# GreatV/oar-ocr

Measured on AMD Instinct MI355X. Metric: images/sec end-to-end PP-OCRv6 det+rec, higher is better.
Workload: dtype f32; 1 GPU; PP-OCRv6-tiny-class det+rec (synthetic-weight graphs: det 447089 params, rec 1135700 params, V=6906), batch=32 synthetic 960x960 pages per GPU, 40 text lines/page; timed region = u8 pages in pageable HOST memory -> oar_ocr_predict -> oar_ocr_decode -> sorted boxes + texts + scores on the host; image_batch_size=32, region_batch_size=256, parallelism=image-parallel x1

## Files before the change

### oar_ocr_amd/build.py

```python
from __future__ import annotations

import os
import subprocess
import sys
from concurrent.futures import ThreadPoolExecutor
from pathlib import Path

HERE = Path(__file__).resolve().parent
CSRC = HERE / "csrc"
LIBDIR = HERE / "lib"
LIB = LIBDIR / "libOarMi355x.so"
SOURCES = ["common.cc", "onnx_parse.cc", "engine.cc", "db_host.cc", "poly_host.cc", "pipeline.cc", "c_api.cc", "ctc_host.cc", "image_decode.cc", "image_misc_decode.cc", "jpeg_decode.cc", "layout.cc", "kernels.hip", "igemm.hip", "igemm_ws_1x1.hip", "igemm_ws_gen.hip", "igemm_ws_x6.hip", "igemm_os_x6.hip", "igemm_ws3.hip", "igemm_rs3_x6.hip", "prepost.hip", "contours.hip", "jpeg.hip", "layout.hip", "dsblock.hip", "dsblock_k3s1.hip", "dsblock_k3s2.hip", "dsblock_k5s1.hip", "dsblock_k5s2.hip", "dsblock_wa_a.hip", "dsblock_wa_b.hip", "dsblock_rs_k3s11.hip", "dsblock_rs_k3s21.hip", "dsblock_rs_k3s12.hip", "dsblock_rs_k3s22.hip", "dsblock_rs_dbg.hip", "dsblock_cs.hip", "dsblock_pc.hip", "dsblock_rs2.hip", "ctc_head_x6.hip", "chain.hip", "attention_x6.hip", "igemm_lk_x6.hip", "index_ops.hip", "sla_decode.hip"]
HIPCC = os.environ.get("HIPCC", "/opt/rocm/bin/hipcc")
FLAGS = ["--offload-arch=gfx950", "-O3", "-std=c++17", "-fPIC", "-ffp-contract=off", "-fno-fast-math",
         "-Wno-unused-result", "-Wno-pass-failed"]
if os.environ.get("OAR_DSB_ABLATIONS"):
    FLAGS.append("-DOAR_DSB_ABLATIONS")


def _stale(out: Path, deps) -> bool:
    if not out.exists():
        return True
    t = out.stat().st_mtime
    return any(Path(d).stat().st_mtime > t for d in deps)


def build_lib(force: bool = False, verbose: bool = False) -> Path:
    LIBDIR.mkdir(exist_ok=True)
    objdir = LIBDIR / "obj"
    objdir.mkdir(exist_ok=True)
    headers = list(CSRC.glob("*.h")) + list(CSRC.glob("*.inc")) + [HERE.parent / "include" / "oar_mi355x.h"]
    jobs = []
    for s in SOURCES:
        src = CSRC / s
        obj = objdir / (s.replace(".", "_") + ".o")
        if force or _stale(obj, [src] + headers):
            jobs.append((src, obj))

    def cc(job):
        src, obj = job
        cmd = [HIPCC] + FLAGS + ["-c", str(src), "-o", str(obj)]
        if verbose:
            print(" ".join(cmd), flush=True)
        r = subprocess.run(cmd, capture_output=True, text=True)
        if r.returncode != 0:
# ... 28 lines not shown
```

### oar_ocr_amd/csrc/engine.cc

```cpp
#include "engine.h"

#include "dsblock.h"

#include <algorithm>
#include <cmath>
#include <cstring>
#include <set>
#include <sstream>

namespace oar {

using k::Act;

static int64_t numel(const std::vector<int64_t>& d) {
    int64_t n = 1;
    for (auto v : d) n *= v;
    return n;
}

Engine::Engine(const uint8_t* onnx, size_t len, int device_id, hipStream_t caller_stream) : device_(device_id) {
    int ndev = 0;
    if (hipGetDeviceCount(&ndev) != hipSuccess || ndev <= 0)
        fail(OAR_DEVICE, "no HIP device visible: libOarMi355x has no CPU fallback");
    OAR_CHECK(device_id >= 0 && device_id < ndev, OAR_DEVICE, "device_id out of range");
// ... 878 lines not shown
    std::vector<int64_t> s(d.size(), 1);
    for (int i = (int)d.size() - 2; i >= 0; --i) s[i] = s[i + 1] * d[i + 1];
    return s;
}

struct Planner {
    Engine& E;
    Plan& P;
    std::map<std::string, TInfo> vals;
    std::map<std::string, int> last_use;
    std::map<std::string, size_t> root_bytes;
    std::map<std::string, size_t> root_off;
    Arena arena;
    int cur = 0;
    std::vector<std::pair<size_t, size_t>> temps;

    Planner(Engine& e, Plan& p) : E(e), P(p) { opset = e.opset_; }

    struct PendingResize {
        Loc xin;
        std::vector<int64_t> dims;
        int N, H, W, C, Ho, Wo, imode, ictm, inm;
        float sh, sw;
        int fh = 0, fw = 0;
    };
    std::map<std::string, PendingResize> pending_resize;
    std::map<std::string, int> sole_consumer;
    void run_resize(const PendingResize& r, Loc yl, int64_t y_off, int y_ld) {
        const PendingResize q = r;
        step([=](const RunCtx& c) { k::resize(c.s, c.at(q.xin), c.mut(yl) + y_off, q.N, q.H, q.W, q.C, q.Ho, q.Wo, q.sh, q.sw, q.imode, q.ictm, q.inm, y_ld); }, 0,
             4.0 * ((double)q.N * q.H * q.W * q.C + (double)q.N * q.Ho * q.Wo * q.C));
    }
    std::map<std::string, const GNode*> pending_convt;
    struct PendingConcat { std::vector<Loc> src; std::vector<int> c; std::vector<int64_t> dims; };
    std::map<std::string, PendingConcat> pending_concat;
    std::map<std::string, int> concat_consumer;
    void emit_concat_gather(const PendingConcat& pc, Loc yl) {
        k::ConcatGatherP gp{};
        gp.n_src = (int)pc.src.size(); gp.N = (int)pc.dims[0]; gp.Ho = (int)pc.dims[2]; gp.Wo = (int)pc.dims[3]; gp.C = (int)pc.dims[1];
        int off = 0;
        for (size_t i = 0; i < pc.src.size(); ++i) { gp.c[i] = pc.c[i]; gp.off[i] = off; gp.fh[i] = 1; gp.fw[i] = 1; off += pc.c[i]; }
        const std::vector<Loc> src = pc.src;
        step([=](const RunCtx& c) {
            k::ConcatGatherP q = gp;
            for (int i = 0; i < q.n_src; ++i) q.x[i] = c.at(src[(size_t)i]);
            k::concat_gather(c.s, q, c.mut(yl));
        }, 0, 8.0 * (double)numel(pc.dims));
    }
    void materialise_concat(const std::string& name) {
        auto it = pending_concat.find(name);
        if (it == pending_concat.end()) return;
        const PendingConcat pc = it->second;
        pending_concat.erase(it);
        vals.erase(name);
        TInfo& y = new_out(name, pc.dims, Layout::CLAST);
        emit_concat_gather(pc, y.loc);
    }
    const PendingResize* peek_pending(const std::string& name) const {
        auto it = pending_resize.find(name);
        return it == pending_resize.end() ? nullptr : &it->second;
    }
    void materialise_pending(const std::string& name) {
        auto ct = pending_convt.find(name);
        if (ct != pending_convt.end()) {
            const GNode* node = ct->second;
            pending_convt.erase(ct);
            vals.erase(name);
            op_convt(*node, false);
            return;
        }
        auto it = pending_resize.find(name);
        if (it == pending_resize.end()) return;
        const PendingResize r = it->second;
        pending_resize.erase(it);
        TInfo& y = new_out(name, r.dims, Layout::CLAST);
        run_resize(r, y.loc, 0, r.C);
    }

    TInfo& get(const std::string& name) {
        if (!pending_resize.empty() || !pending_convt.empty()) materialise_pending(name);
// ... 613 lines not shown
            int64_t th = std::max<int64_t>((oh - 1) * sh + (kh - 1) * dh + 1 - H, 0), tw = std::max<int64_t>((ow - 1) * sw + (kw - 1) * dw + 1 - W, 0);
            if (ap == "SAME_UPPER") { pt = th / 2; pb = th - pt; pl = tw / 2; pr = tw - pl; }
            else { pb = th / 2; pt = th - pb; pr = tw / 2; pl = tw - pr; }
        }
    }

    void op_conv(const GNode& n) {
        if (n.in.size() > 3 && !n.in[3].empty()) {
            TInfo xg = get(n.in[0]), gt = get(n.in[3]);
            const TInfo& wg = get(n.in[1]);
            bool ok = xg.dims.size() == 4 && !xg.host_int && !gt.host_int && wg.ht && wg.ht->dims.size() == 4 && gt.loc.kind != Loc::NONE && n.residual.empty();
            if (ok) {
                const int64_t N = xg.dims[0], C = xg.dims[1], HW = xg.dims[2] * xg.dims[3];
                ok = numel(gt.dims) == N * C && gt.dims.size() >= 2 && gt.dims[0] == N && gt.dims[1] == C && wg.ht->dims[1] == C && C % 8 == 0 &&
                     k::conv_igemm_se_ok(N * HW, (int)C, (int)wg.ht->dims[0], (int)HW);
            }
            if (!ok) {
                GNode mul;
                mul.op = "Mul"; mul.in = {n.in[0], n.in[3]}; mul.out = {n.out[0] + "::se"};
                op_binary(mul, 2);
                GNode c2 = n;
                c2.in.resize(3);
                c2.in[0] = mul.out[0];
                op_conv(c2);
                return;
            }
        }
        PendingConcat msrc;
        {
            auto pit = pending_concat.find(n.in[0]);
            if (pit != pending_concat.end()) {
                auto wi = E.inits_.find(n.in.size() > 1 ? n.in[1] : std::string());
                const std::vector<int64_t>& pd = pit->second.dims;
                const bool still_ok = wi != E.inits_.end() && wi->second.dims.size() == 4 && wi->second.dims[2] == 1 && wi->second.dims[3] == 1 && n.residual.empty() &&
                                      !(n.in.size() > 3 && !n.in[3].empty()) && n.out.size() == 1 &&
                                      k::conv_msrc_ok((long)(pd[0] * pd[2] * pd[3]), (int)pd[1], (int)wi->second.dims[0]);
                if (getenv("OAR_DEBUG_CONCAT")) fprintf(stderr, "  conv %s reads pending concat: still_ok=%d (w4=%d res=%d gate=%d nout=%zu)\n", n.out[0].c_str(), (int)still_ok, (int)(wi != E.inits_.end() && wi->second.dims.size() == 4), (int)!n.residual.empty(), (int)(n.in.size() > 3 && !n.in[3].empty()), n.out.size());
                if (still_ok) { msrc = pit->second; TInfo keep = vals[n.in[0]]; pending_concat.erase(pit); vals[n.in[0]] = keep; }
            }
        }
        TInfo x = get(n.in[0]);
        OAR_CHECK(x.dims.size() == 4, OAR_UNSUPPORTED_OP, "Conv: only 2-D convolutions are supported");
        const TInfo& wt = get(n.in[1]);
        OAR_CHECK(wt.ht, OAR_UNSUPPORTED_OP, "Conv: weights must be an initializer");
        const HostTensor& W = *wt.ht;
        OAR_CHECK(W.dims.size() == 4 && W.dims[0] > 0 && W.dims[1] > 0 && W.dims[2] > 0 && W.dims[3] > 0, OAR_MODEL_LOAD, "Conv: weight must be rank 4 with positive dims at " + n.out[0]);
        int64_t N = x.dims[0], Cin = x.dims[1], H = x.dims[2], Wd = x.dims[3];
        int64_t Cout = W.dims[0], kh = W.dims[2], kw = W.dims[3], g = n.ai("group", 1);
        OAR_CHECK(g >= 1 && W.dims[1] * g == Cin && Cout % g == 0, OAR_SHAPE_MISMATCH, "Conv: weight/input channel mismatch at " + n.out[0]);
        if (has_input(n, 2)) { const TInfo& bt = get(n.in[2]); OAR_CHECK(bt.ht && (int64_t)bt.ht->f.size() == Cout, OAR_MODEL_LOAD, "Conv: bias must be an f32 initializer of Cout elements at " + n.out[0]); }
        auto st = n.ais("strides"), dl = n.ais("dilations");
        int64_t sh = st.size() == 2 ? st[0] : 1, sw = st.size() == 2 ? st[1] : 1;
        int64_t dh = dl.size() == 2 ? dl[0] : 1, dw = dl.size() == 2 ? dl[1] : 1;
        int64_t pt, pl, pb, pr;
        get_pads(n, H, Wd, kh, kw, sh, sw, dh, dw, pt, pl, pb, pr);
        int64_t Ho = (H + pt + pb - dh * (kh - 1) - 1) / sh + 1, Wo = (Wd + pl + pr - dw * (kw - 1) - 1) / sw + 1;
        if (x.u8_stem) {
            OAR_CHECK(g == 1 && Cin == 3 && kh * kw * 3 <= 128 && n.residual.empty(), OAR_INTERNAL, "run_stem on a graph whose first node is not an RGB stem");
            const float* sb = has_input(n, 2) ? get(n.in[2]).loc.cptr : nullptr;
            TInfo& ys = new_out(n.out[0], {N, Cout, Ho, Wo}, Layout::CLAST);
            k::ConvP sp{};
            sp.N = (int)N; sp.H = (int)H; sp.W = (int)Wd; sp.Cin = 3; sp.Ho = (int)Ho; sp.Wo = (int)Wo; sp.Cout = (int)Cout;
            sp.kh = (int)kh; sp.kw = (int)kw; sp.sh = (int)sh; sp.sw = (int)sw; sp.pt = (int)pt; sp.pl = (int)pl; sp.dh = (int)dh; sp.dw = (int)dw;
            sp.groups = 1; sp.act = n.act; sp.bias = sb; sp.y_ld = (int)Cout; sp.convt2x2 = 0;
            sp.w = conv_weight_direct(n, W);
            const Loc ysl = ys.loc;
            step([=](const RunCtx& c) {
// ... 98 lines not shown
            gate = get(n.in[3]).loc;
        }
        const bool has_gate = gate.kind != Loc::NONE;
        double flops = 2.0 * N * Ho * Wo * Cout * (Cin / g) * kh * kw;
        double bytes = 4.0 * (N * H * Wd * Cin + N * Ho * Wo * Cout * (has_res ? 2 : 1) + numel(W.dims));
        if (n.out.size() > 1) {
            const int tiles = kind == 1 ? k::conv_dw_gap_tiles(p) : 0;
            if (tiles > 0 && Cout <= 1024 && n.ai("gap_raw", 0) != 0) {
                TInfo& gy = new_out(n.out[1], {N, (int64_t)tiles * Cout, 1, 1}, Layout::CLAST);
                gy.gap_tiles = tiles; gy.gap_hw = (int)(Ho * Wo);
                const Loc part = gy.loc;
                step([=](const RunCtx& c) {
                    k::ConvP q = p;
                    q.x = c.at(xin); q.y = c.mut(yl); q.residual = has_res ? c.at(res) : nullptr; q.gap_part = c.mut(part);
                    k::conv_dw(c.s, q);
                }, flops, bytes + 4.0 * N * tiles * Cout);
                return;
            }
            if (tiles > 0 && Cout <= 1024) {
                TInfo& gy = new_out(n.out[1], {N, Cout, 1, 1}, Layout::CLAST);
                const Loc gl = gy.loc, part = alloc_temp((size_t)N * tiles * Cout * sizeof(float));
                const int hw = (int)(Ho * Wo);
                step([=](const RunCtx& c) {
                    k::ConvP q = p;
                    q.x = c.at(xin); q.y = c.mut(yl); q.residual = has_res ? c.at(res) : nullptr; q.gap_part = c.mut(part);
                    k::conv_dw(c.s, q);
                }, flops, bytes + 4.0 * N * tiles * Cout);
                step([=](const RunCtx& c) { k::global_avgpool_finish(c.s, c.at(part), c.mut(gl), (int)N, tiles, (int)Cout, hw); }, 0, 4.0 * N * tiles * Cout);
                return;
            }
        }
        const bool from_concat = !msrc.src.empty();
        OAR_CHECK(!from_concat || (kind == 0 && p.w_fmt == k::IGEMM_W_X6), OAR_INTERNAL, "Conv: deferred concat in front of a layer that is not on the bf16x6 kernels");
        auto run = [=](const RunCtx& c) {
            k::ConvP q = p;
            q.y = c.mut(yl); q.residual = has_res ? c.at(res) : nullptr; q.se = has_gate ? c.at(gate) : nullptr;
            if (from_concat) {
                q.x = nullptr; q.n_msrc = (int)msrc.src.size();
                for (int i = 0; i < q.n_msrc; ++i) { q.msrc[i] = c.at(msrc.src[(size_t)i]); q.msrc_c[i] = msrc.c[(size_t)i]; }
            } else {
                q.x = c.at(xin);
            }
            if (kind == 3) {
                const int ng = p.groups, cgi = p.Cin / ng, ogi = p.Cout / ng;
                for (int gi = 0; gi < ng; ++gi) {
                    k::ConvP r = q;
                    r.groups = 1; r.Cin = cgi; r.Cout = ogi; r.x_ld = p.Cin;
                    r.x = q.x + (size_t)gi * cgi; r.y = q.y + (size_t)gi * ogi; r.w = wgrp[(size_t)gi];
                    r.bias = q.bias ? q.bias + (size_t)gi * ogi : nullptr;
                    r.residual = q.residual ? q.residual + (size_t)gi * ogi : nullptr;
                    k::conv_igemm(c.s, r);
                }
                return;
            }
            if (kind == 4) {
                int c0 = 0;
                for (size_t i = 0; i < slices3.size(); ++i) {
                    k::ConvP r = q;
                    r.Cin = slices3[i]; r.x_ld = p.Cin; r.x = q.x + c0; r.w = wgrp[i]; r.accum = i > 0 ? 1 : 0;
                    if (i > 0) r.bias = nullptr;
                    if (i + 1 < slices3.size()) r.act = k::Act{};
                    k::conv_igemm(c.s, r);
                    c0 += slices3[i];
                }
                return;
            }
// ... 912 lines not shown
        }
        std::string mode = n.as("mode", "nearest"), ctm = n.as("coordinate_transformation_mode", "half_pixel"), nm = n.as("nearest_mode", "round_prefer_floor");
        int imode = mode == "nearest" ? 0 : 1;
        OAR_CHECK(mode == "nearest" || mode == "linear", OAR_UNSUPPORTED_OP, "Resize: mode " + mode);
        int ictm = ctm == "asymmetric" ? 0 : ctm == "half_pixel" ? 1 : ctm == "align_corners" ? 2 : ctm == "pytorch_half_pixel" ? 3 : -1;
        OAR_CHECK(ictm >= 0, OAR_UNSUPPORTED_OP, "Resize: coordinate_transformation_mode " + ctm);
        int inm = nm == "floor" ? 0 : nm == "round_prefer_floor" ? 1 : nm == "round_prefer_ceil" ? 2 : 3;
        static const bool defer_on = [] { const char* e = getenv("OAR_DEFER_RESIZE"); return !e || atoi(e) != 0; }();
        if (defer_on && imode == 0 && x.layout == Layout::CLAST && sole_consumer.count(n.out[0])) {
            PendingResize r;
            r.xin = x.loc; r.dims = {x.dims[0], x.dims[1], Ho, Wo};
            r.N = (int)x.dims[0]; r.H = (int)H; r.W = (int)W; r.C = (int)x.dims[1]; r.Ho = (int)Ho; r.Wo = (int)Wo;
            r.imode = imode; r.ictm = ictm; r.inm = inm; r.sh = sh; r.sw = sw;
            auto factor = [&](int in, int out, float scale) {
                if (in <= 0 || out % in != 0) return 0;
                const int f = out / in;
                for (int o = 0; o < out; ++o) if (k::resize_nearest_index(o, scale, in, out, ictm, inm) != o / f) return 0;
                return f;
            };
            r.fh = factor(r.H, r.Ho, sh); r.fw = factor(r.W, r.Wo, sw);
            if (!r.fh || !r.fw) r.fh = r.fw = 0;
            pending_resize[n.out[0]] = r;
            TInfo t;
            t.dims = r.dims; t.layout = Layout::CLAST; t.root = "";
            vals[n.out[0]] = t;
            return;
        }
        Loc xin = to_clast_loc(x);
        TInfo& y = new_out(n.out[0], {x.dims[0], x.dims[1], Ho, Wo}, Layout::CLAST);
        Loc yl = y.loc;
        int N = (int)x.dims[0], C = (int)x.dims[1];
        step([=](const RunCtx& c) { k::resize(c.s, c.at(xin), c.mut(yl), N, (int)H, (int)W, C, (int)Ho, (int)Wo, sh, sw, imode, ictm, inm, C); }, 0,
             4.0 * (numel(x.dims) + numel(y.dims)));
    }

    void op_concat(const GNode& n) {
        bool absorb = false;
        if (!pending_resize.empty()) {
            int64_t axis0 = n.ai("axis", 0);
            bool ok = true, any = false;
            int64_t total_c = 0;
            for (auto& s : n.in) {
                const PendingResize* pr = peek_pending(s);
                any = any || pr;
                auto it = vals.find(s);
                if (it == vals.end() || it->second.dims.size() != 4 || it->second.layout != Layout::CLAST || it->second.host_int) { ok = false; break; }
                if ((it->second.dims[1] & 3) != 0) ok = false;
                total_c += it->second.dims[1];
            }
            absorb = any && ok && (axis0 == 1 || axis0 == -3) && (total_c & 3) == 0;
            if (!absorb) for (auto& s : n.in) materialise_pending(s);
        }
        std::vector<TInfo> xs;
        for (auto& s : n.in) { auto it = vals.find(s); xs.push_back(absorb && peek_pending(s) ? it->second : get(s)); }
        bool all_host = true, any_host = false, any_f = false;
        for (auto& t : xs) { all_host = all_host && host_evaluable(t) && t.dims.size() <= 1; any_host = any_host || t.host_int; any_f = any_f || float_like(t); }
        if (all_host && any_host) {
            std::vector<double> v;
            for (auto& t : xs) { std::vector<double> e = host_values(t); v.insert(v.end(), e.begin(), e.end()); }
            set_host(n.out[0], {(int64_t)v.size()}, v, any_f);
            return;
        }
        int r = (int)xs[0].dims.size();
        int64_t axis = n.ai("axis", 0);
        if (axis < 0) axis += r;
        bool clast = false;
// ... 8 lines not shown
            for (int i = 0; i < pax; ++i) outer *= pod[i];
            for (int i = pax + 1; i < r; ++i) inner *= pod[i];
            std::vector<Loc> ins;
            for (size_t i = 0; i < xs.size(); ++i) ins.push_back(absorb && peek_pending(n.in[i]) ? Loc() : to_clast_loc(xs[i]));
            int64_t coff = 0, total = pod[pax] * inner;
            bool plain = !absorb && r == 4 && inner == 1 && xs.size() >= 3 && (od[1] & 3) == 0;
            for (auto& t : xs) plain = plain && t.dims.size() == 4 && (t.dims[1] & 3) == 0;
            static const bool defer_on = [] { const char* e = getenv("OAR_CONCAT_DEFER"); return !(e && e[0] == '0'); }();
            if (getenv("OAR_DEBUG_CONCAT")) fprintf(stderr, "concat %s: plain=%d absorb=%d r=%d inner=%ld n=%zu consumer=%d\n", n.out[0].c_str(), (int)plain, (int)absorb, r, (long)inner, xs.size(), concat_consumer.count(n.out[0]) ? concat_consumer[n.out[0]] : -1);
            if (plain && defer_on && xs.size() <= 8 && concat_consumer.count(n.out[0])) {
                const GNode& cn = E.nodes_[concat_consumer[n.out[0]]];
                auto wi = E.inits_.find(cn.in.size() > 1 ? cn.in[1] : std::string());
                auto attr_ok = [&](const char* a, int64_t want) { auto v = cn.ais(a); for (auto e : v) if (e != want) return false; return true; };
                bool ok = wi != E.inits_.end() && wi->second.dims.size() == 4 && wi->second.dims[2] == 1 && wi->second.dims[3] == 1 && wi->second.dims[1] == od[1] && cn.ai("group", 1) == 1 &&
                          attr_ok("strides", 1) && attr_ok("pads", 0) && attr_ok("dilations", 1) && cn.residual.empty() && !(cn.in.size() > 3 && !cn.in[3].empty()) &&
                          cn.as("auto_pad", "NOTSET") == "NOTSET";
                for (auto& t : xs) ok = ok && t.layout == Layout::CLAST && (t.dims[1] & 7) == 0 && t.dims[0] == od[0] && t.dims[2] == od[2] && t.dims[3] == od[3] && !t.host_int;
                if (getenv("OAR_DEBUG_CONCAT")) {
                    fprintf(stderr, "  ok before msrc check = %d (K=%ld N=%ld) res=%d gate=%d autopad=%s\n", (int)ok, (long)od[1], wi != E.inits_.end() ? (long)wi->second.dims[0] : -1L, (int)!cn.residual.empty(), (int)(cn.in.size() > 3 && !cn.in[3].empty()), cn.as("auto_pad", "NOTSET").c_str());
                    for (auto& t : xs) fprintf(stderr, "    src layout=%d C=%ld host=%d\n", (int)(t.layout == Layout::CLAST), (long)t.dims[1], (int)t.host_int);
                }
                ok = ok && k::conv_msrc_ok((long)(od[0] * od[2] * od[3]), (int)od[1], (int)wi->second.dims[0]) && (wi->second.dims[0] & 3) == 0;
                if (ok) {
                    PendingConcat pc;
                    for (size_t i = 0; i < xs.size(); ++i) { pc.src.push_back(ins[i]); pc.c.push_back((int)xs[i].dims[1]); }
                    pc.dims = od;
                    TInfo t;
                    t.dims = od; t.layout = Layout::CLAST;
                    vals[n.out[0]] = t;
                    pending_concat[n.out[0]] = std::move(pc);
                    return;
                }
            }
            TInfo& y = new_out(n.out[0], od, Layout::CLAST);
            Loc yl = y.loc;
            if ((absorb || plain) && r == 4 && inner == 1 && xs.size() <= 8) {
                static const bool gather_on = [] { const char* e = getenv("OAR_CONCAT_GATHER"); return !(e && e[0] == '0'); }();
                bool ok = gather_on;
                for (size_t i = 0; ok && i < xs.size(); ++i) {
                    const PendingResize* pr = peek_pending(n.in[i]);
                    if (pr) ok = pr->fh > 0 && pr->fw > 0 && pr->imode == 0 && pr->Ho == od[2] && pr->Wo == od[3] && pr->H * pr->fh == pr->Ho && pr->W * pr->fw == pr->Wo && pr->N == od[0];
                    else ok = xs[i].dims[0] == od[0] && xs[i].dims[2] == od[2] && xs[i].dims[3] == od[3];
                }
                if (ok) {
                    k::ConcatGatherP gp{};
                    std::vector<Loc> src(xs.size());
                    gp.n_src = (int)xs.size(); gp.N = (int)od[0]; gp.Ho = (int)od[2]; gp.Wo = (int)od[3]; gp.C = (int)od[1];
                    double bytes = 4.0 * (double)numel(od);
                    for (size_t i = 0; i < xs.size(); ++i) {
                        const PendingResize* pr = peek_pending(n.in[i]);
                        src[i] = pr ? pr->xin : ins[i];
                        gp.c[i] = (int)xs[i].dims[1]; gp.off[i] = (int)coff; gp.fh[i] = pr ? pr->fh : 1; gp.fw[i] = pr ? pr->fw : 1;
                        bytes += 4.0 * (double)numel(xs[i].dims) / (gp.fh[i] * gp.fw[i]);
                        coff += xs[i].dims[1];
                    }
                    for (auto& nm : n.in) pending_resize.erase(nm);
                    step([=](const RunCtx& c) {
                        k::ConcatGatherP q = gp;
                        for (int i = 0; i < q.n_src; ++i) q.x[i] = c.at(src[(size_t)i]);
                        k::concat_gather(c.s, q, c.mut(yl));
                    }, 0, bytes);
                    return;
                }
            }
            for (size_t i = 0; i < xs.size(); ++i) {
                int64_t w = xs[i].dims[axis] * inner;
// ... 623 lines not shown
                const GNode& n = E.nodes_[i];
                for (auto& s : n.in) if (!s.empty()) { auto& u = uses[s]; ++u.first; u.second = i; }
                if (!n.residual.empty()) { auto& u = uses[n.residual]; ++u.first; u.second = i; }
            }
            for (int i = 0; i < (int)E.nodes_.size(); ++i) {
                const GNode& n = E.nodes_[i];
                if ((n.op != "Resize" && n.op != "ConvTranspose") || n.out.empty() || n.in.empty()) continue;
                auto u = uses.find(n.out[0]);
                if (u == uses.end() || u->second.first != 1) continue;
                if (std::find(E.output_names_.begin(), E.output_names_.end(), n.out[0]) != E.output_names_.end()) continue;
                sole_consumer[n.out[0]] = u->second.second;
                int& l = lu[n.in[0]];
                l = std::max(l, u->second.second);
            }
        }
        concat_consumer.clear();
        {
            std::map<std::string, std::pair<int, int>> uses;
            for (int i = 0; i < (int)E.nodes_.size(); ++i) {
                const GNode& n = E.nodes_[i];
                for (auto& s : n.in) if (!s.empty()) { auto& u = uses[s]; ++u.first; u.second = i; }
                if (!n.residual.empty()) { auto& u = uses[n.residual]; ++u.first; u.second = i; }
            }
            for (int i = 0; i < (int)E.nodes_.size(); ++i) {
                const GNode& n = E.nodes_[i];
                if (n.op != "Concat" || n.out.empty() || n.in.size() < 3) continue;
                auto u = uses.find(n.out[0]);
                if (u == uses.end() || u->second.first != 1) continue;
                if (std::find(E.output_names_.begin(), E.output_names_.end(), n.out[0]) != E.output_names_.end()) continue;
                const GNode& cn = E.nodes_[u->second.second];
                if (cn.op != "Conv" || cn.in.empty() || cn.in[0] != n.out[0]) continue;
                concat_consumer[n.out[0]] = u->second.second;
                for (auto& sname : n.in) { int& l = lu[sname]; l = std::max(l, u->second.second); }
            }
        }
        for (int i = (int)E.nodes_.size() - 1; i >= 0; --i) {
            const GNode& n = E.nodes_[i];
            if (!alias_ops.count(n.op) || n.in.empty()) continue;
            int m = lu.count(n.in[0]) ? lu[n.in[0]] : i;
            for (auto& o : n.out) if (lu.count(o)) m = std::max(m, lu[o]);
            lu[n.in[0]] = m;
        }
        last_use = lu;
    }

    int read_after(const std::string& v) const { auto it = last_use.find(v); return it == last_use.end() ? -1 : it->second; }
    std::string node_desc(int i) const {
        const GNode& g = E.nodes_[(size_t)i];
        return "node " + std::to_string(i) + " (" + g.op + " -> " + (g.out.empty() ? std::string("?") : g.out[0]) + ")";
    }
    int checked_upto = -1;
    void check_release(const std::vector<std::string>& dead, int i) {
        for (auto& d : dead) {
            auto al = root_aliases.find(d);
            if (al == root_aliases.end()) continue;
            for (auto& v : al->second) {
                auto vi = vals.find(v);
                if (vi == vals.end() || vi->second.root != d || vi->second.loc.kind != Loc::ARENA) continue;
                const int r = read_after(v);
                OAR_CHECK(r <= i, OAR_INTERNAL, "plan liveness: " + node_desc(i) + " frees root '" + d + "' but '" + v + "' lives in it and is read " +
                          (r >= (1 << 30) ? std::string("as a graph output") : "at node " + std::to_string(r)));
            }
        }
        for (int j = checked_upto + 1; j <= i; ++j) {
            for (auto& o : E.nodes_[(size_t)j].out) {
                auto vi = vals.find(o);
// ... 462 lines not shown
```

### oar_ocr_amd/csrc/kernels.h

```cpp
#pragma once
#include <hip/hip_runtime.h>

#include <cstdint>
#include <vector>

namespace oar {
namespace k {

enum ActKind : int { ACT_NONE = 0, ACT_RELU, ACT_HSWISH, ACT_HSIGMOID, ACT_SIGMOID, ACT_SWISH, ACT_LEAKY, ACT_CLIP, ACT_TANH, ACT_GELU_ERF,
                     ACT_ERF, ACT_SQRT, ACT_EXP, ACT_ABS, ACT_NEG, ACT_RECIP, ACT_LOG, ACT_GELU_TANH, ACT_SOFTPLUS, ACT_FLOOR, ACT_CEIL, ACT_ROUND, ACT_NOT };
struct Act {
    int kind = ACT_NONE;
    float alpha = 0.f, beta = 0.f;
};

struct ConvP {
    int N, H, W, Cin;
    int Ho, Wo, Cout;
    int kh, kw, sh, sw, pt, pl, dh, dw, groups;
    Act act;
    const float* x;
    const float* w;
    const float* bias;
    const float* residual;
    float* y;
    int y_ld;
    int convt2x2;
    int w_fmt;
    float* ctc_part;
    int ctc_valid;
    const float* se;
    int res_up;
    int n_msrc;
    const float* msrc[8];
    int msrc_c[8];
    int accum;
    int x_ld;
    float* gap_part;
};
enum : int { IGEMM_W_K16 = 0, IGEMM_W_X6 = 1, IGEMM_W_X6RS = 2, IGEMM_W_X6CS = 3 };

void conv_igemm(hipStream_t s, const ConvP& p);
int igemm_weight_format(long M, int K, int N, bool is1x1, int Cin = 0, long same3x3_px = 0, bool lk_ok = false);
bool conv_lk_x6_eligible(int kh, int kw, int sh, int sw, int pt, int pl, int dh, int dw, int H, int W, int Ho, int Wo, int Cin, int Cout, int y_ld, long M);
bool conv_grouped_x6_ok(long M, int K, int N, int Cin);
bool conv_msrc_ok(long M, int K, int N);
std::vector<int> conv3x3_n16_slices(long M, int Cin, int Cout, long img_px, int y_ld);
bool conv_igemm_se_ok(long M, int K, int N, int hw);
void conv_dw(hipStream_t s, const ConvP& p);
int conv_dw_gap_tiles(const ConvP& p);
void global_avgpool_finish(hipStream_t s, const float* part, float* y, int N, int tiles, int C, int hw);
void conv_direct(hipStream_t s, const ConvP& p);
struct StemImg { const uint8_t* ptr; int32_t w; int32_t pad; };
struct StemU8 { const uint8_t* pages[32]; int src[3]; float alpha[3], beta[3]; const StemImg* dev = nullptr; };
void conv_smallcin_u8(hipStream_t s, const ConvP& p, const StemU8& st);
struct ConvT2Pair {
    const float* x; float* y;
    const float *w1, *b1, *w2, *b2;
    int N, H, W, C0, C1, C2;
    Act act1, act2;
};
bool convt2x2_pair_supported(int C0, int C1, int C2);
void convt2x2_pair(hipStream_t s, const ConvT2Pair& p);
void convt_direct(hipStream_t s, const ConvP& p);

struct PoolP {
    int N, H, W, C, Ho, Wo, kh, kw, sh, sw, pt, pl;
    int pb, pr;
    int is_max, count_include_pad;
    const float* x;
    float* y;
};
void pool2d(hipStream_t s, const PoolP& p);
int global_avgpool_splits(int N, int HW, int C);
void global_avgpool(hipStream_t s, const float* x, float* y, int N, int HW, int C, float* partial = nullptr);

int resize_nearest_index(int o, float scale, int in, int out, int ctm, int nearest_mode);
void binary_upsampled(hipStream_t s, const float* a, const float* b, float* y, int N, int Ho, int Wo, int C, int fh, int fw, int op);
void resize(hipStream_t s, const float* x, float* y, int N, int H, int W, int C, int Ho, int Wo, float scale_h,
            float scale_w, int mode, int ctm, int nearest_mode, int y_ld);
// ... 91 lines not shown
```

Before: 2503 images/sec.

## Fuse concat and nearest upsample into the 3x3 row-streaming conv input gather

Adds a row-streaming 3x3 conv kernel (Cout<=16, bf16x6 MFMA) that reads up to four concat sources directly. Nearest-neighbour upsampled sources are read at their low resolution by shifting coordinates. The planner defers the concat and any pending resizes when the sole consumer is such a 3x3 conv, and extends source lifetimes to match. This skips materialising the upsampled tensors and the concatenated tensor in the detection neck/head. It costs a new kernel with per-lane source selection and extra planner complexity.

```diff
diff --git a/oar_ocr_amd/build.py b/oar_ocr_amd/build.py
--- a/oar_ocr_amd/build.py
+++ b/oar_ocr_amd/build.py
@@ -10,7 +10,7 @@
 CSRC = HERE / "csrc"
 LIBDIR = HERE / "lib"
 LIB = LIBDIR / "libOarMi355x.so"
-SOURCES = ["common.cc", "onnx_parse.cc", "engine.cc", "db_host.cc", "poly_host.cc", "pipeline.cc", "c_api.cc", "ctc_host.cc", "image_decode.cc", "image_misc_decode.cc", "jpeg_decode.cc", "layout.cc", "kernels.hip", "igemm.hip", "igemm_ws_1x1.hip", "igemm_ws_gen.hip", "igemm_ws_x6.hip", "igemm_os_x6.hip", "igemm_ws3.hip", "igemm_rs3_x6.hip", "prepost.hip", "contours.hip", "jpeg.hip", "layout.hip", "dsblock.hip", "dsblock_k3s1.hip", "dsblock_k3s2.hip", "dsblock_k5s1.hip", "dsblock_k5s2.hip", "dsblock_wa_a.hip", "dsblock_wa_b.hip", "dsblock_rs_k3s11.hip", "dsblock_rs_k3s21.hip", "dsblock_rs_k3s12.hip", "dsblock_rs_k3s22.hip", "dsblock_rs_dbg.hip", "dsblock_cs.hip", "dsblock_pc.hip", "dsblock_rs2.hip", "ctc_head_x6.hip", "chain.hip", "attention_x6.hip", "igemm_lk_x6.hip", "index_ops.hip", "sla_decode.hip"]
+SOURCES = ["common.cc", "onnx_parse.cc", "engine.cc", "db_host.cc", "poly_host.cc", "pipeline.cc", "c_api.cc", "ctc_host.cc", "image_decode.cc", "image_misc_decode.cc", "jpeg_decode.cc", "layout.cc", "kernels.hip", "igemm.hip", "igemm_ws_1x1.hip", "igemm_ws_gen.hip", "igemm_ws_x6.hip", "igemm_os_x6.hip", "igemm_ws3.hip", "igemm_rs3_x6.hip", "igemm_rs3g_x6.hip", "prepost.hip", "contours.hip", "jpeg.hip", "layout.hip", "dsblock.hip", "dsblock_k3s1.hip", "dsblock_k3s2.hip", "dsblock_k5s1.hip", "dsblock_k5s2.hip", "dsblock_wa_a.hip", "dsblock_wa_b.hip", "dsblock_rs_k3s11.hip", "dsblock_rs_k3s21.hip", "dsblock_rs_k3s12.hip", "dsblock_rs_k3s22.hip", "dsblock_rs_dbg.hip", "dsblock_cs.hip", "dsblock_pc.hip", "dsblock_rs2.hip", "ctc_head_x6.hip", "chain.hip", "attention_x6.hip", "igemm_lk_x6.hip", "index_ops.hip", "sla_decode.hip"]
 HIPCC = os.environ.get("HIPCC", "/opt/rocm/bin/hipcc")
 FLAGS = ["--offload-arch=gfx950", "-O3", "-std=c++17", "-fPIC", "-ffp-contract=off", "-fno-fast-math",
          "-Wno-unused-result", "-Wno-pass-failed"]
diff --git a/oar_ocr_amd/csrc/engine.cc b/oar_ocr_amd/csrc/engine.cc
--- a/oar_ocr_amd/csrc/engine.cc
+++ b/oar_ocr_amd/csrc/engine.cc
@@ -934,20 +934,24 @@
              4.0 * ((double)q.N * q.H * q.W * q.C + (double)q.N * q.Ho * q.Wo * q.C));
     }
     std::map<std::string, const GNode*> pending_convt;
-    struct PendingConcat { std::vector<Loc> src; std::vector<int> c; std::vector<int64_t> dims; };
+    struct PendingConcat { std::vector<Loc> src; std::vector<int> c; std::vector<int64_t> dims; std::vector<int> fh, fw; bool conv3 = false; };
     std::map<std::string, PendingConcat> pending_concat;
     std::map<std::string, int> concat_consumer;
     void emit_concat_gather(const PendingConcat& pc, Loc yl) {
         k::ConcatGatherP gp{};
         gp.n_src = (int)pc.src.size(); gp.N = (int)pc.dims[0]; gp.Ho = (int)pc.dims[2]; gp.Wo = (int)pc.dims[3]; gp.C = (int)pc.dims[1];
         int off = 0;
-        for (size_t i = 0; i < pc.src.size(); ++i) { gp.c[i] = pc.c[i]; gp.off[i] = off; gp.fh[i] = 1; gp.fw[i] = 1; off += pc.c[i]; }
+        double bytes = 4.0 * (double)numel(pc.dims);
+        for (size_t i = 0; i < pc.src.size(); ++i) {
+            gp.c[i] = pc.c[i]; gp.off[i] = off; gp.fh[i] = pc.fh.empty() ? 1 : pc.fh[i]; gp.fw[i] = pc.fw.empty() ? 1 : pc.fw[i]; off += pc.c[i];
+            bytes += 4.0 * (double)(pc.dims[0] * pc.dims[2] * pc.dims[3]) * pc.c[i] / (gp.fh[i] * gp.fw[i]);
+        }
         const std::vector<Loc> src = pc.src;
         step([=](const RunCtx& c) {
             k::ConcatGatherP q = gp;
             for (int i = 0; i < q.n_src; ++i) q.x[i] = c.at(src[(size_t)i]);
             k::concat_gather(c.s, q, c.mut(yl));
-        }, 0, 8.0 * (double)numel(pc.dims));
+        }, 0, bytes);
     }
     void materialise_concat(const std::string& name) {
         auto it = pending_concat.find(name);
@@ -1627,7 +1631,11 @@
             if (pit != pending_concat.end()) {
                 auto wi = E.inits_.find(n.in.size() > 1 ? n.in[1] : std::string());
                 const std::vector<int64_t>& pd = pit->second.dims;
-                const bool still_ok = wi != E.inits_.end() && wi->second.dims.size() == 4 && wi->second.dims[2] == 1 && wi->second.dims[3] == 1 && n.residual.empty() &&
+                const PendingConcat& pq = pit->second;
+                const bool still_ok = pq.conv3 ? (wi != E.inits_.end() && wi->second.dims.size() == 4 && wi->second.dims[2] == 3 && wi->second.dims[3] == 3 && n.residual.empty() &&
+                                                  !(n.in.size() > 3 && !n.in[3].empty()) && n.out.size() == 1 && n.ai("group", 1) == 1 &&
+                                                  k::conv3x3_n16_gather_ok((int)pd[0], (int)pd[2], (int)pd[3], (int)wi->second.dims[0], (int)pq.c.size(), pq.c.data(), pq.fh.data(), pq.fw.data())) :
+                                      wi != E.inits_.end() && wi->second.dims.size() == 4 && wi->second.dims[2] == 1 && wi->second.dims[3] == 1 && n.residual.empty() &&
                                       !(n.in.size() > 3 && !n.in[3].empty()) && n.out.size() == 1 &&
                                       k::conv_msrc_ok((long)(pd[0] * pd[2] * pd[3]), (int)pd[1], (int)wi->second.dims[0]);
                 if (getenv("OAR_DEBUG_CONCAT")) fprintf(stderr, "  conv %s reads pending concat: still_ok=%d (w4=%d res=%d gate=%d nout=%zu)\n", n.out[0].c_str(), (int)still_ok, (int)(wi != E.inits_.end() && wi->second.dims.size() == 4), (int)!n.residual.empty(), (int)(n.in.size() > 3 && !n.in[3].empty()), n.out.size());
@@ -1792,6 +1800,26 @@
         }
         const bool from_concat = !msrc.src.empty();
         OAR_CHECK(!from_concat || (kind == 0 && p.w_fmt == k::IGEMM_W_X6), OAR_INTERNAL, "Conv: deferred concat in front of a layer that is not on the bf16x6 kernels");
+        if (from_concat && msrc.conv3) {
+            OAR_CHECK(kh == 3 && kw == 3 && sh == 1 && sw == 1 && pt == 1 && pl == 1 && pb == 1 && pr == 1 && dh == 1 && dw == 1 && Ho == H && Wo == Wd && g == 1 && !has_res && !has_gate, OAR_INTERNAL,
+                      "Conv: a concat deferred for the row-streaming 3x3 kernel in front of another layer");
+            k::Conv3GatherP gq{};
+            gq.n_src = (int)msrc.src.size(); gq.N = (int)N; gq.H = (int)H; gq.W = (int)Wd; gq.Cout = (int)Cout; gq.y_ld = (int)Cout;
+            gq.w = p.w; gq.bias = bias; gq.act = n.act;
+            double src_floats = 0;
+            for (int i = 0; i < gq.n_src; ++i) {
+                gq.c[i] = msrc.c[(size_t)i]; gq.fh[i] = msrc.fh[(size_t)i]; gq.fw[i] = msrc.fw[(size_t)i];
+                src_floats += (double)(N * H * Wd) * gq.c[i] / (gq.fh[i] * gq.fw[i]);
+            }
+            const std::vector<Loc> srcs = msrc.src;
+            step([=](const RunCtx& c) {
+                k::Conv3GatherP q = gq;
+                for (int i = 0; i < q.n_src; ++i) q.x[i] = c.at(srcs[(size_t)i]);
+                q.y = c.mut(yl);
+                k::conv3x3_n16_gather(c.s, q);
+            }, flops, 4.0 * (src_floats + (double)(N * Ho * Wo * Cout) + (double)numel(W.dims)));
+            return;
+        }
         auto run = [=](const RunCtx& c) {
             k::ConvP q = p;
             q.y = c.mut(yl); q.residual = has_res ? c.at(res) : nullptr; q.se = has_gate ? c.at(gate) : nullptr;
@@ -2770,6 +2798,28 @@
         int N = (int)x.dims[0], C = (int)x.dims[1];
         step([=](const RunCtx& c) { k::resize(c.s, c.at(xin), c.mut(yl), N, (int)H, (int)W, C, (int)Ho, (int)Wo, sh, sw, imode, ictm, inm, C); }, 0,
              4.0 * (numel(x.dims) + numel(y.dims)));
+    }
+
+    bool conv3_reads_sources(const GNode& cn, const GNode& n, const std::vector<TInfo>& xs, const std::vector<int64_t>& od, PendingConcat& pc) {
+        auto wi = E.inits_.find(cn.in.size() > 1 ? cn.in[1] : std::string());
+        auto attr_ok = [&](const char* a, int64_t want) { auto v = cn.ais(a); for (auto e : v) if (e != want) return false; return true; };
+        if (cn.op != "Conv" || cn.in.empty() || cn.in[0] != n.out[0] || wi == E.inits_.end() || wi->second.dims.size() != 4 || wi->second.dims[2] != 3 || wi->second.dims[3] != 3 ||
+            wi->second.dims[1] != od[1] || cn.ai("group", 1) != 1 || !attr_ok("strides", 1) || !attr_ok("pads", 1) || cn.ais("pads").size() != 4 || !attr_ok("dilations", 1) ||
+            !cn.residual.empty() || (cn.in.size() > 3 && !cn.in[3].empty()) || cn.out.size() != 1 || cn.as("auto_pad", "NOTSET") != "NOTSET") return false;
+        int c[4], fh[4], fw[4];
+        for (size_t i = 0; i < xs.size(); ++i) {
+            const PendingResize* pr = peek_pending(n.in[i]);
+            if (pr) {
+                if (!(pr->fh > 0 && pr->fw > 0 && pr->imode == 0 && pr->Ho == od[2] && pr->Wo == od[3] && pr->H * pr->fh == pr->Ho && pr->W * pr->fw == pr->Wo && pr->N == od[0])) return false;
+            } else if (xs[i].layout != Layout::CLAST || xs[i].host_int || xs[i].loc.kind == Loc::NONE || xs[i].dims.size() != 4 || xs[i].dims[0] != od[0] || xs[i].dims[2] != od[2] || xs[i].dims[3] != od[3]) {
+                return false;
+            }
+            c[i] = (int)xs[i].dims[1]; fh[i] = pr ? pr->fh : 1; fw[i] = pr ? pr->fw : 1;
+        }
+        if (od[0] * od[2] * od[3] >= ((int64_t)1 << 31) || !k::conv3x3_n16_gather_ok((int)od[0], (int)od[2], (int)od[3], (int)wi->second.dims[0], (int)xs.size(), c, fh, fw)) return false;
+        pc.c.assign(c, c + xs.size()); pc.fh.assign(fh, fh + xs.size()); pc.fw.assign(fw, fw + xs.size());
+        pc.dims = od; pc.conv3 = true;
+        return true;
     }
 
     void op_concat(const GNode& n) {
@@ -2844,6 +2894,22 @@
                     return;
                 }
             }
+            if ((absorb || plain) && defer_on && r == 4 && inner == 1 && xs.size() >= 2 && xs.size() <= 4 && concat_consumer.count(n.out[0])) {
+                const GNode& cn = E.nodes_[concat_consumer[n.out[0]]];
+                PendingConcat pc;
+                if (conv3_reads_sources(cn, n, xs, od, pc)) {
+                    for (size_t i = 0; i < xs.size(); ++i) {
+                        const PendingResize* pr = peek_pending(n.in[i]);
+                        pc.src.push_back(pr ? pr->xin : ins[i]);
+                    }
+                    for (auto& nm : n.in) pending_resize.erase(nm);
+                    TInfo t;
+                    t.dims = od; t.layout = Layout::CLAST;
+                    vals[n.out[0]] = t;
+                    pending_concat[n.out[0]] = std::move(pc);
+                    return;
+                }
+            }
             TInfo& y = new_out(n.out[0], od, Layout::CLAST);
             Loc yl = y.loc;
             if ((absorb || plain) && r == 4 && inner == 1 && xs.size() <= 8) {
@@ -3533,6 +3599,13 @@
                 if (cn.op != "Conv" || cn.in.empty() || cn.in[0] != n.out[0]) continue;
                 concat_consumer[n.out[0]] = u->second.second;
                 for (auto& sname : n.in) { int& l = lu[sname]; l = std::max(l, u->second.second); }
+                auto cw = E.inits_.find(cn.in.size() > 1 ? cn.in[1] : std::string());
+                const bool reader3 = cw != E.inits_.end() && cw->second.dims.size() == 4 && cw->second.dims[2] == 3 && cw->second.dims[3] == 3 && cw->second.dims[0] <= 16;
+                for (auto& sname : n.in) {
+                    if (!reader3 || !sole_consumer.count(sname)) continue;
+                    for (const GNode& rn : E.nodes_)
+                        if (rn.op == "Resize" && !rn.out.empty() && rn.out[0] == sname && !rn.in.empty()) { int& l = lu[rn.in[0]]; l = std::max(l, u->second.second); }
+                }
             }
         }
         for (int i = (int)E.nodes_.size() - 1; i >= 0; --i) {
diff --git a/oar_ocr_amd/csrc/igemm_rs3g_x6.hip b/oar_ocr_amd/csrc/igemm_rs3g_x6.hip
--- /dev/null
+++ b/oar_ocr_amd/csrc/igemm_rs3g_x6.hip
@@ -0,0 +1,242 @@
+#include <hip/hip_ext.h>
+
+#include "igemm_dev.h"
+
+namespace oar {
+namespace k {
+
+typedef unsigned g3_u32x4 __attribute__((ext_vector_type(4)));
+typedef unsigned g3_u32x2 __attribute__((ext_vector_type(2)));
+typedef __bf16 g3_bf16x8 __attribute__((ext_vector_type(8)));
+
+struct Rs3gP {
+    const float* src[4];
+    int sc[4], lfh[4], lfw[4];
+    int n_src;
+    float* y; const float4* w; const float* bias;
+    int N, H, W, Cin, Cout, y_ld;
+    int act; float alpha, beta;
+    int R, segs, tiles_x, items, per_xcd;
+    unsigned y_bytes;
+};
+
+namespace {
+constexpr unsigned kG3OobSt = 0x80000000u, kG3Zero = 0x40000000u;
+constexpr int kG3IW = 18, kG3PxB = 144, kG3PlB = kG3IW * kG3PxB, kG3RowB = 3 * kG3PlB, kG3Waves = 6;
+
+__device__ __forceinline__ g3_u32x4 g3_lds4(unsigned off) {
+    return *reinterpret_cast<const __attribute__((address_space(3))) g3_u32x4*>((__attribute__((address_space(3))) const char*)nullptr + off);
+}
+__device__ __forceinline__ void g3_lds_w2(unsigned off, g3_u32x2 v) {
+    *reinterpret_cast<__attribute__((address_space(3))) g3_u32x2*>((__attribute__((address_space(3))) char*)nullptr + off) = v;
+}
+
+template <int CC32>
+__global__ __launch_bounds__(kG3Waves * 64, 2) void conv3x3_n16_x6g_kernel(Rs3gP p) {
+    constexpr int QPP = CC32 * 8;
+    constexpr int NU = kG3IW * QPP;
+    constexpr int NJ = (NU + 63) / 64;
+    constexpr int KC = 9 * CC32;
+    static_assert(64 % QPP == 0, "a lane keeps its channel quad over the loads of a row");
+    extern __shared__ float4 g3_lds[];
+    const int tid = threadIdx.x, lane = tid & 63;
+    const int wave = __builtin_amdgcn_readfirstlane(tid >> 6);
+    const int g = lane >> 4, n = lane & 15;
+    const unsigned ring0 = (unsigned)(wave * 3 * kG3RowB);
+
+    g3_u32x4 wreg[KC][2];
+#pragma unroll
+    for (int kc = 0; kc < KC; ++kc)
+#pragma unroll
+        for (int s = 0; s < 2; ++s) {
+            const float4 v = p.w[(kc * 3 + s) * 64 + lane];
+            wreg[kc][s] = (g3_u32x4){__float_as_uint(v.x), __float_as_uint(v.y), __float_as_uint(v.z), __float_as_uint(v.w)};
+        }
+    constexpr unsigned kWl = (unsigned)(kG3Waves * 3 * kG3RowB);
+    for (int i = tid; i < KC * 64; i += kG3Waves * 64) g3_lds[(kWl >> 4) + i] = p.w[((i >> 6) * 3 + 2) * 64 + (i & 63)];
+    __syncthreads();
+    const float4 bq = (p.bias && g * 4 < p.Cout) ? *reinterpret_cast<const float4*>(p.bias + g * 4) : make_float4(0.f, 0.f, 0.f, 0.f);
+
+    const int cq = lane & (QPP - 1);
+    const float* sbase = p.src[0];
+    int cs = p.sc[0], c0 = 0, lfh = p.lfh[0], lfw = p.lfw[0];
+    {
+        int acc_c = p.sc[0];
+#pragma unroll
+        for (int i = 1; i < 4; ++i) {
+            const bool hit = i < p.n_src && cq * 4 >= acc_c;
+            sbase = hit ? p.src[i] : sbase; cs = hit ? p.sc[i] : cs; c0 = hit ? acc_c : c0; lfh = hit ? p.lfh[i] : lfh; lfw = hit ? p.lfw[i] : lfw;
+            acc_c += p.sc[i];
+        }
+    }
+    const unsigned srow_bytes = (unsigned)((p.W >> lfw) * cs * 4);
+    const long simg_bytes = (long)(p.H >> lfh) * srow_bytes;
+    const char* const slane = reinterpret_cast<const char*>(sbase) + (cq * 4 - c0) * 4;
+
+    const int xcd = (int)(blockIdx.x & 7), wgx = (int)(blockIdx.x >> 3), wgs = (int)(gridDim.x >> 3);
+    const int b0 = xcd * p.per_xcd, b1 = min(p.items, b0 + p.per_xcd);
+    const int J = wgs * kG3Waves, j0 = wgx * kG3Waves + wave;
+    const int orow_bytes = p.W * p.y_ld * 4;
+    const __amdgpu_buffer_rsrc_t ysrc = __builtin_amdgcn_make_buffer_rsrc(p.y, 0, (int)p.y_bytes, 0x00020000);
+    const unsigned rd_lane = (unsigned)(n * kG3PxB + g * 16);
+
+    for (int item = b0 + j0; item < b1; item += J) {
+        const int tx = item % p.tiles_x, q_ = item / p.tiles_x, seg = q_ % p.segs, img = q_ / p.segs;
+        const int o_begin = seg * p.R, o_end = min(p.H, o_begin + p.R);
+        const int x0 = tx * 16 - 1;
+        const char* const ximg = slane + (long)img * simg_bytes;
+        unsigned src[NJ], dst[NJ];
+#pragma unroll
+        for (int u = 0; u < NJ; ++u) {
+            const int q = u * 64 + lane, px = q / QPP;
+            const int xc = min(max(x0 + px, 0), p.W - 1);
+            src[u] = (unsigned)(((xc >> lfw) * cs) * 4);
+            dst[u] = q < NU ? (unsigned)(px * kG3PxB + cq * 8) | ((unsigned)(x0 + px) < (unsigned)p.W ? 0u : kG3Zero) : 0xFFFFFFFFu;
+        }
+        g3_u32x4 in[NJ];
+        auto load_row = [&](int y, g3_u32x4 (&in)[NJ]) __attribute__((always_inline)) {
+            const int yc = min(max(y, 0), p.H - 1);
+            const unsigned ro = (unsigned)(yc >> lfh) * srow_bytes;
+#pragma unroll
+            for (int u = 0; u < NJ; ++u) in[u] = *reinterpret_cast<const g3_u32x4*>(ximg + (unsigned)(ro + src[u]));
+        };
+        auto put_row = [&](unsigned slot, const g3_u32x4 (&in)[NJ], bool rok) __attribute__((always_inline)) {
+#pragma unroll
+            for (int u = 0; u < NJ; ++u) {
+                const unsigned keep = (rok && !(dst[u] & kG3Zero)) ? 0xFFFFFFFFu : 0u;
+                unsigned hb[4], mb[4], lb[4];
+#pragma unroll
+                for (int e = 0; e < 4; ++e) {
+                    const unsigned ux = in[u][e] & keep;
+                    const float xf = __uint_as_float(ux);
+                    const float r1 = xf - __uint_as_float(ux & 0xFFFF0000u);
+                    const unsigned u1 = __float_as_uint(r1);
+                    const float r2 = r1 - __uint_as_float(u1 & 0xFFFF0000u);
+                    hb[e] = ux; mb[e] = u1; lb[e] = __float_as_uint(r2);
+                }
+                if (dst[u] != 0xFFFFFFFFu) {
+                    const unsigned a = slot + (dst[u] & ~kG3Zero);
+                    g3_lds_w2(a, (g3_u32x2){__builtin_amdgcn_perm(hb[1], hb[0], 0x07060302u), __builtin_amdgcn_perm(hb[3], hb[2], 0x07060302u)});
+                    g3_lds_w2(a + kG3PlB, (g3_u32x2){__builtin_amdgcn_perm(mb[1], mb[0], 0x07060302u), __builtin_amdgcn_perm(mb[3], mb[2], 0x07060302u)});
+                    g3_lds_w2(a + 2 * kG3PlB, (g3_u32x2){__builtin_amdgcn_perm(lb[1], lb[0], 0x07060302u), __builtin_amdgcn_perm(lb[3], lb[2], 0x07060302u)});
+                }
+            }
+        };
+        auto row_ok = [&](int y) { return (unsigned)y < (unsigned)p.H; };
+        {
+            g3_u32x4 in1[NJ], in2[NJ];
+            load_row(o_begin - 1, in);
+            load_row(o_begin, in1);
+            load_row(o_begin + 1, in2);
+            put_row(ring0, in, row_ok(o_begin - 1));
+            put_row(ring0 + (unsigned)kG3RowB, in1, row_ok(o_begin));
+            put_row(ring0 + (unsigned)(2 * kG3RowB), in2, row_ok(o_begin + 1));
+        }
+        int s0 = 0;
+        const int ox = tx * 16 + n;
+        const unsigned st_lane = (ox < p.W && g * 4 < p.Cout) ? (unsigned)((ox * p.y_ld + g * 4) * 4) : kG3OobSt;
+        unsigned st_row = (unsigned)((img * p.H + o_begin) * orow_bytes);
+#pragma unroll 1
+        for (int r = o_begin; r < o_end; ++r) {
+            load_row(r + 2, in);
+            f32x4 acc[6];
+            acc[5] = (f32x4){bq.x, bq.y, bq.z, bq.w};
+            acc[0] = acc[1] = acc[2] = acc[3] = acc[4] = (f32x4){0.f, 0.f, 0.f, 0.f};
+            unsigned rd = ring0 + rd_lane;
+            unsigned slot_of[3];
+#pragma unroll
+            for (int kh = 0; kh < 3; ++kh) slot_of[kh] = (unsigned)((s0 + kh >= 3 ? s0 + kh - 3 : s0 + kh) * kG3RowB);
+            g3_u32x4 xs[3][4];
+            auto fetch = [&](int kc, g3_u32x4 (&dstv)[4]) __attribute__((always_inline)) {
+                const int kh = kc / (3 * CC32), kw = (kc / CC32) % 3, c = kc % CC32;
+#pragma unroll
+                for (int s_ = 0; s_ < 3; ++s_) dstv[s_] = g3_lds4(rd + slot_of[kh] + (unsigned)(s_ * kG3PlB + kw * kG3PxB + c * 64));
+                dstv[3] = g3_lds4(rd - rd_lane - ring0 + kWl + (unsigned)(kc * 1024 + lane * 16));
+            };
+            fetch(0, xs[0]);
+            fetch(1, xs[1]);
+#pragma unroll
+            for (int kc = 0; kc < KC; ++kc) {
+                if (kc + 2 < KC) fetch(kc + 2, xs[(kc + 2) % 3]);
+                constexpr int WPL[6] = {1, 2, 0, 1, 0, 0}, XPL[6] = {1, 0, 2, 0, 1, 0};
+#pragma unroll
+                for (int t = 0; t < 6; ++t)
+                    acc[t] = __builtin_amdgcn_mfma_f32_16x16x32_bf16(__builtin_bit_cast(g3_bf16x8, WPL[t] == 2 ? xs[kc % 3][3] : wreg[kc][WPL[t] == 2 ? 0 : WPL[t]]), __builtin_bit_cast(g3_bf16x8, xs[kc % 3][XPL[t]]), acc[t], 0, 0, 0);
+                asm("" : "+v"(rd) : "v"(xs[kc % 3][2]));
+            }
+            f32x4 o = ((((acc[0] + acc[1]) + acc[2]) + acc[3]) + acc[4]) + acc[5];
+            g3_u32x4 v;
+#pragma unroll
+            for (int e = 0; e < 4; ++e) v[e] = __float_as_uint(apply_act(o[e] + 0.f, p.act, p.alpha, p.beta));
+            asm volatile("s_waitcnt lgkmcnt(0)" ::: "memory");
+            put_row(ring0 + (unsigned)(s0 * kG3RowB), in, row_ok(r + 2));
+            __builtin_amdgcn_raw_buffer_store_b128(v, ysrc, (int)(st_lane + st_row), 0, 0);
+            st_row += (unsigned)orow_bytes;
+            s0 = s0 + 1 == 3 ? 0 : s0 + 1;
+        }
+    }
+}
+}
+
+static bool gather_shape_ok(int N, int H, int W, int Cout, int n_src, const int* c, const int* fh, const int* fw) {
+    if (n_src < 2 || n_src > 4 || H <= 0 || W <= 0) return false;
+    int Cin = 0;
+    for (int i = 0; i < n_src; ++i) {
+        if (c[i] <= 0 || (c[i] & 3) != 0) return false;
+        for (int f : {fh[i], fw[i]}) if (f != 1 && f != 2 && f != 4 && f != 8) return false;
+        if (H % fh[i] != 0 || W % fw[i] != 0) return false;
+        Cin += c[i];
+    }
+    return conv3x3_n16_x6_eligible((long)N * H * W, Cin, Cout, (long)H * W, 4 * Cout);
+}
+bool conv3x3_n16_gather_ok(int N, int H, int W, int Cout, int n_src, const int* c, const int* fh, const int* fw) {
+    const char* e = getenv("OAR_CONCAT_DEFER3");
+    return !(e && e[0] == '0') && gather_shape_ok(N, H, W, Cout, n_src, c, fh, fw);
+}
+
+void conv3x3_n16_gather(hipStream_t s, const Conv3GatherP& g) {
+    OAR_CHECK(gather_shape_ok(g.N, g.H, g.W, g.Cout, g.n_src, g.c, g.fh, g.fw) && g.y_ld == g.Cout, OAR_INTERNAL, "conv3x3_n16_gather: not a layer conv3x3_n16_gather_ok accepts");
+    Rs3gP p{};
+    int Cin = 0;
+    double src_floats = 0;
+    for (int i = 0; i < g.n_src; ++i) {
+        p.src[i] = g.x[i]; p.sc[i] = g.c[i];
+        p.lfh[i] = __builtin_ctz((unsigned)g.fh[i]); p.lfw[i] = __builtin_ctz((unsigned)g.fw[i]);
+        Cin += g.c[i];
+        src_floats += (double)g.N * (g.H / g.fh[i]) * (g.W / g.fw[i]) * g.c[i];
+    }
+    p.n_src = g.n_src;
+    p.y = g.y; p.w = reinterpret_cast<const float4*>(g.w); p.bias = g.bias;
+    p.N = g.N; p.H = g.H; p.W = g.W; p.Cin = Cin; p.Cout = g.Cout; p.y_ld = g.y_ld;
+    p.act = g.act.kind; p.alpha = g.act.alpha; p.beta = g.act.beta;
+    p.tiles_x = (g.W + 15) / 16;
+    const long waves = 256L * kG3Waves;
+    double best = 1e30;
+    for (int R = std::min(g.H, 4); R <= g.H; ++R) {
+        const int segs = (g.H + R - 1) / R;
+        const long items = (long)g.N * segs * p.tiles_x;
+        const long rounds = (items + waves - 1) / waves;
+        const double cost = (double)rounds * (R + 2.5);
+        if (cost < best - 1e-9) { best = cost; p.R = R; p.segs = segs; p.items = (int)items; }
+    }
+    p.per_xcd = (p.items + 7) / 8;
+    const long M = (long)g.N * g.H * g.W;
+    p.y_bytes = (unsigned)(M * g.y_ld * 4);
+    const size_t lds = (size_t)kG3Waves * 3 * kG3RowB + (size_t)9 * (Cin / 32) * 1024;
+    char pname[96];
+    const char* cls = "conv_rs3_x6";
+    if (Profiler::get().detail) {
+        snprintf(pname, sizeof pname, "conv_igemm_rs3_x6 M=%ld K=%d N=%d k3x3 s1 gather%d", M, 9 * Cin, g.Cout, g.n_src);
+        cls = pname;
+    }
+    ProfScope ps(s, cls, 4.0 * (src_floats + (double)M * g.Cout + 9.0 * Cin * g.Cout), 2.0 * (double)M * 9 * Cin * g.Cout);
+    auto launch = [&](auto kernel) {
+        OAR_MAX_LDS_ONCE(kernel, 160 * 1024);
+        hipLaunchKernelGGL(kernel, dim3(256), dim3(kG3Waves * 64), lds, s, p);
+    };
+    if (Cin == 64) launch(conv3x3_n16_x6g_kernel<2>);
+    else launch(conv3x3_n16_x6g_kernel<1>);
+}
+
+}
+}
diff --git a/oar_ocr_amd/csrc/kernels.h b/oar_ocr_amd/csrc/kernels.h
--- a/oar_ocr_amd/csrc/kernels.h
+++ b/oar_ocr_amd/csrc/kernels.h
@@ -46,6 +46,9 @@
 bool conv_grouped_x6_ok(long M, int K, int N, int Cin);
 bool conv_msrc_ok(long M, int K, int N);
 std::vector<int> conv3x3_n16_slices(long M, int Cin, int Cout, long img_px, int y_ld);
+struct Conv3GatherP { const float* x[4]; int c[4], fh[4], fw[4]; int n_src, N, H, W, Cout, y_ld; const float* w; const float* bias; float* y; Act act; };
+bool conv3x3_n16_gather_ok(int N, int H, int W, int Cout, int n_src, const int* c, const int* fh, const int* fw);
+void conv3x3_n16_gather(hipStream_t s, const Conv3GatherP& p);
 bool conv_igemm_se_ok(long M, int K, int N, int hw);
 void conv_dw(hipStream_t s, const ConvP& p);
 int conv_dw_gap_tiles(const ConvP& p);
```

After: 2561 images/sec, median of 6. 1.02x the previous value.
